# AuCson/DSP-Speech-Recognition

Hardware: NVIDIA B200
Metric: audio-sec/sec of MFCC+delta+pitch+endpoint (full front-end), ragged 0.5-5 s utterances, per-GPU LPT shards (higher is better)
Workload: dtype f32

## Files before the change

### dsp-speech-recognition_b200/csrc/fft_regs.h

```cpp
#pragma once
#include "simt.h"

namespace dspfe {

struct cpx2 { float2 re, im; };

DEVFN cpx2 cadd(cpx2 a, cpx2 b) { cpx2 r; r.re = f2add(a.re, b.re); r.im = f2add(a.im, b.im); return r; }
DEVFN cpx2 csub(cpx2 a, cpx2 b) { cpx2 r; r.re = f2sub(a.re, b.re); r.im = f2sub(a.im, b.im); return r; }
DEVFN cpx2 cmuls(cpx2 a, float wr, float wi) {
    cpx2 r;
    r.re = f2fmas(a.re, wr, f2muls(a.im, -wi));
    r.im = f2fmas(a.re, wi, f2muls(a.im, wr));
    return r;
}
DEVFN cpx2 cmul_negi(cpx2 a) { cpx2 r; r.re = a.im; r.im = f2neg(a.re); return r; }

DEVFN void dft4(cpx2& a, cpx2& b, cpx2& c, cpx2& d) {
    cpx2 t0 = cadd(a, c), t1 = csub(a, c), t2 = cadd(b, d), t3 = cmul_negi(csub(b, d));
    a = cadd(t0, t2); c = csub(t0, t2); b = cadd(t1, t3); d = csub(t1, t3);
}

DEVFN void dft16(cpx2 (&x)[16]) {
    const float c1 = 0.92387953251128674f, s1 = 0.38268343236508977f, r2 = 0.70710678118654752f;
#pragma unroll
    for (int nb = 0; nb < 4; ++nb) dft4(x[nb], x[4 + nb], x[8 + nb], x[12 + nb]);
    x[5] = cmuls(x[5], c1, -s1);
    { cpx2 t = x[6]; x[6].re = f2muls(f2add(t.re, t.im), r2); x[6].im = f2muls(f2sub(t.im, t.re), r2); }
    x[7] = cmuls(x[7], s1, -c1);
    { cpx2 t = x[9]; x[9].re = f2muls(f2add(t.re, t.im), r2); x[9].im = f2muls(f2sub(t.im, t.re), r2); }
    x[10] = cmul_negi(x[10]);
    { cpx2 t = x[11]; x[11].re = f2muls(f2sub(t.im, t.re), r2); x[11].im = f2muls(f2add(t.re, t.im), -r2); }
    x[13] = cmuls(x[13], s1, -c1);
    { cpx2 t = x[14]; x[14].re = f2muls(f2sub(t.im, t.re), r2); x[14].im = f2muls(f2add(t.re, t.im), -r2); }
    x[15] = cmuls(x[15], -c1, s1);
#pragma unroll
    for (int ka = 0; ka < 4; ++ka) dft4(x[4 * ka], x[4 * ka + 1], x[4 * ka + 2], x[4 * ka + 3]);
#pragma unroll
    for (int a = 0; a < 4; ++a)
#pragma unroll
        for (int b = a + 1; b < 4; ++b) { cpx2 t = x[4 * a + b]; x[4 * a + b] = x[4 * b + a]; x[4 * b + a] = t; }
}

DEVFN cpx2 shfl_xor_c(cpx2 a, int m) {
    cpx2 r;
    r.re.x = simt::shfl32_xor(a.re.x, m); r.re.y = simt::shfl32_xor(a.re.y, m);
    r.im.x = simt::shfl32_xor(a.im.x, m); r.im.y = simt::shfl32_xor(a.im.y, m);
    return r;
}

template <bool W32IMM = false>
DEVFN void fft512(cpx2 (&x)[16], float2* scr, const float2* tws, const float2* w32s, int lane) {
    dft16(x);
    const int q = lane >> 4, ll = lane & 15;
    const float sg = q ? -1.f : 1.f;
#pragma unroll
    for (int k1 = 0; k1 < 16; ++k1) {
        const float kC[16] = {1.0f, 0.98078528f, 0.923879533f, 0.831469612f, 0.707106781f, 0.555570233f, 0.382683432f, 0.195090322f, 6.123234e-17f, -0.195090322f, -0.382683432f, -0.555570233f, -0.707106781f, -0.831469612f, -0.923879533f, -0.98078528f};
        const float kS[16] = {-0.0f, -0.195090322f, -0.382683432f, -0.555570233f, -0.707106781f, -0.831469612f, -0.923879533f, -0.98078528f, -1.0f, -0.98078528f, -0.923879533f, -0.831469612f, -0.707106781f, -0.555570233f, -0.382683432f, -0.195090322f};
        const float2 w = W32IMM ? make_float2(q ? kC[k1] : 1.f, q ? kS[k1] : 0.f) : w32s[2 * k1 + q];
        const cpx2 u = cmuls(x[k1], w.x, w.y);
        const cpx2 v = shfl_xor_c(u, 16);
        cpx2 d; d.re = f2fmas(u.re, sg, v.re); d.im = f2fmas(u.im, sg, v.im);
        const float2 t = tws[k1 * 32 + lane];
        x[k1] = cmuls(d, t.x, t.y);
    }
    float2* tile = scr + q * (16 * 17);
#pragma unroll
    for (int k1 = 0; k1 < 16; ++k1) tile[k1 * 17 + ll] = x[k1].re;
    simt::warp_sync();
#pragma unroll
    for (int n2 = 0; n2 < 16; ++n2) x[n2].re = tile[ll * 17 + n2];
    simt::warp_sync();
#pragma unroll
    for (int k1 = 0; k1 < 16; ++k1) tile[k1 * 17 + ll] = x[k1].im;
    simt::warp_sync();
#pragma unroll
    for (int n2 = 0; n2 < 16; ++n2) x[n2].im = tile[ll * 17 + n2];
    simt::warp_sync();
    dft16(x);
}

}
```

### dsp-speech-recognition_b200/csrc/pitch_kernel.cuh

```cuda
#pragma once
#include <math.h>
#include <stdint.h>

#include "simt.h"
#include "fft_regs.h"
#ifndef DSPFE_EMU
#include <cuda_fp16.h>
#endif

#ifndef DSP_HD
#ifdef __CUDACC__
#define DSP_HD __host__ __device__ inline
#else
#define DSP_HD inline
#endif
#endif

namespace dspfe {

constexpr int kPitchFft = 1024;
constexpr int kCepLen = 512;
constexpr int kCepCols = 200;
constexpr int kAcrLags = 180;
constexpr int kMinLag = 20;
// ... 398 lines not shown
    int u, nf; int64_t g0;
    slot_unit(p, h0, kClipRun, lane, u, g0, nf);
    if (lane == 0) p.run_desc[h0 / kClipRun] = make_int4((int)(g0 & 0xffffffffll), (int)(g0 >> 32), nf, u);
    if (nf == 0) return;
    const int Ld = p.ds_len[u];
    const int kf0 = (int)(g0 - p.frame_off[u]) * step;
    const int fit = ((kClipDecCap - L) / step + 1) & ~1;
#pragma unroll 1
    for (int j0 = 0; j0 < nf; j0 += fit) {
        const int nj = nf - j0 < fit ? nf - j0 : fit;
        const int span = (nj - 1) * step + L;
        simt::warp_sync();
        FrameCursor c = frame_cursor(p, g0 + j0, u, lane, true, stage, span, kClipStageBytes);
        const int rows = (((span + 31) >> 5) + 3) & ~3;
        const bool pre = p.pre_hi != 0.f || p.pre_lo != 0.f;
        if (p.in_f32) { if (pre) decimate_span<true, true>(p, c, ds_idx, dec, lane, rows); else decimate_span<true, false>(p, c, ds_idx, dec, lane, rows); }
        else { if (pre) decimate_span<false, true>(p, c, ds_idx, dec, lane, rows); else decimate_span<false, false>(p, c, ds_idx, dec, lane, rows); }
        simt::warp_sync();
#pragma unroll 1
        for (int j = j0; j < j0 + nj; j += 2) {
            const bool hasB = j + 1 < nf && j + 1 < j0 + nj;
            float xa[NT], xb[NT], fa = 0.f, fb = 0.f;
            const int base = (j - j0) * step;
            const int cnta = L < Ld - (kf0 + j * step) ? L : Ld - (kf0 + j * step);
            const int cntb = hasB ? (L < Ld - (kf0 + (j + 1) * step) ? L : Ld - (kf0 + (j + 1) * step)) : 0;
#pragma unroll
            for (int t = 0; t < NT; ++t) {
                const int n = 32 * t + lane;
                const float va = n < cnta ? dec[base + n] : 0.f, vb = n < cntb ? dec[base + step + n] : 0.f;
                xa[t] = va; xb[t] = vb; fa += fabsf(va); fb += fabsf(vb);
            }
            if (p.frame_amp) {
                double sa = (double)fa, sb = (double)fb;
#pragma unroll
                for (int m = 16; m >= 1; m >>= 1) { sa += shfl32_xor_f64(sa, m); sb += shfl32_xor_f64(sb, m); }
                if (lane == 0) { p.frame_amp[g0 + j] = sa; if (hasB) p.frame_amp[g0 + j + 1] = sb; }
            }
            float2 med = make_float2(0.f, 0.f);
            if (p.do_clip) med = I16 ? warp_median_nonneg2_i16<NT>(xa, xb, L, lane) : warp_median_nonneg2<NT>(xa, xb, L, lane);
            float2* dst = p.clip + ((h0 + j) >> 1) * 512;
#pragma unroll
            for (int t = 0; t < 16; ++t) {
                float2 o = make_float2(0.f, 0.f);
                if (t < NT && lane + 32 * t < L) {
                    o.x = p.do_clip ? clip_value(xa[t < NT ? t : 0], med.x) : xa[t < NT ? t : 0];
                    o.y = p.do_clip ? clip_value(xb[t < NT ? t : 0], med.y) : xb[t < NT ? t : 0];
                }
                dst[32 * t + lane] = o;
            }
        }
    }
}

template <int MODE>
DEVFN void pitch_fft_pair(const PitchParams& p, int64_t h0, int64_t g0, bool hasB, unsigned char* wsm, const float2* tws, const float2* w32s) {
    const int lane = simt::tid() & 31;
    float2* scr = reinterpret_cast<float2*>(wsm);
    float4* park = reinterpret_cast<float4*>(scr + kWarpScr);
    float2* xs = p.clip + (h0 >> 1) * 512;
    const float2* modA = p.tab + kTabMod;
    const float2* HeB = p.tab + kTabHe;
    const float2* HoB = p.tab + kTabHo;
    const int L = p.frame_len;
    cpx2 x[16];
    const float2 zero2 = make_float2(0.f, 0.f);
    const float inv1024 = 1.0f / 1024.0f;
    constexpr int kStages = MODE == 0 ? 5 : 8;
#pragma unroll 1
    for (int st = 0; st < kStages; ++st) {
        const bool inv = MODE == 0 ? (st == 2 || st == 4) : (st & 1);
        const bool load = MODE == 0 ? st <= 1 : !(st & 1);
        const bool loadmod = MODE == 0 ? st == 1 : (st == 2 || st == 6);
        if (load) {
#pragma unroll
            for (int t = 0; t < 16; ++t) {
                const float2 xv = xs[32 * t + lane];
                float2 m = make_float2(1.f, 0.f);
                if (loadmod) m = ldg(modA + 32 * t + lane);
                x[t].re = f2muls(xv, m.x); x[t].im = f2muls(xv, m.y);
            }
        }
        if (inv) {
#pragma unroll
            for (int t = 0; t < 16; ++t) x[t].im = f2neg(x[t].im);
        }
        fft512<true>(x, scr, tws, w32s, lane);
        if (inv) {
#pragma unroll
            for (int t = 0; t < 16; ++t) x[t].im = f2neg(x[t].im);
        }
        const bool mulH = MODE == 0 ? st <= 1 : (st == 0 || st == 2);
        const bool mulM = MODE == 0 ? st == 2 : st == 3;
        if (mulH || mulM) {
            const float2* T = mulM ? modA : ((MODE == 0 ? st == 0 : st == 0) ? HeB : HoB);
            const float sr = mulM ? (MODE == 0 ? inv1024 : 1.f) : ((MODE == 0 && st == 0) ? 0.5f : 1.f);
            const float si = mulM ? -sr : sr;
#pragma unroll
            for (int t = 0; t < 16; ++t) { const float2 h = ldg(T + 32 * t + lane); x[t] = cmuls(x[t], h.x * sr, h.y * si); }
        }
        if (MODE == 0) {
            if (st == 0) {
#pragma unroll
                for (int t = 0; t < 16; ++t) park[32 * t + lane] = make_float4(x[t].re.x, x[t].re.y, x[t].im.x, x[t].im.y);
            } else if (st == 3) {
#pragma unroll
                for (int t = 0; t < 16; ++t) {
                    const float4 pk = park[32 * t + lane];
                    const float2 yr = f2add(x[t].re, make_float2(pk.x, pk.y)), yi = f2add(x[t].im, make_float2(pk.z, pk.w));
                    const float2 s2 = f2fma(yi, yi, f2mul(yr, yr));
                    x[t].re = make_float2(0.5f * dsp_fast_logf(s2.x), 0.5f * dsp_fast_logf(s2.y));
                    x[t].im = zero2;
                }
            } else if (st == 4) {
                const float inv512 = 1.0f / 512.0f;
                float* rowa = p.rows + g0 * p.row_len;
                float* rowb = rowa + p.row_len;
#pragma unroll
                for (int t = 0; t < 16; ++t) {
                    const int n = 32 * t + lane;
                    if (n < p.row_len) {
                        const float2 s2 = f2fma(x[t].im, x[t].im, f2mul(x[t].re, x[t].re));
                        rowa[n] = dsp_fast_sqrtf(s2.x) * inv512;
                        if (hasB) rowb[n] = dsp_fast_sqrtf(s2.y) * inv512;
                    }
                }
            }
        } else {
            if (st == 1) {
#pragma unroll
                for (int t = 0; t < 16; ++t) park[32 * t + lane] = make_float4(x[t].re.x, x[t].re.y, x[t].im.x, x[t].im.y);
            } else if (st == 3) {
#pragma unroll
                for (int t = 0; t < 16; ++t) {
                    const float4 pk = park[32 * t + lane];
                    const float2 yr = f2add(x[t].re, make_float2(pk.x, pk.y)), yi = f2add(x[t].im, make_float2(pk.z, pk.w));
                    const float2 s2 = f2fma(yi, yi, f2mul(yr, yr));
                    const bool in = 32 * t + lane < L;
                    xs[32 * t + lane] = make_float2(in ? dsp_fast_sqrtf(s2.x) * inv1024 : 0.f, in ? dsp_fast_sqrtf(s2.y) * inv1024 : 0.f);
                }
            } else if (st == 4 || st == 6) {
#pragma unroll
                for (int t = 0; t < 16; ++t) { x[t].re = f2fma(x[t].im, x[t].im, f2mul(x[t].re, x[t].re)); x[t].im = zero2; }
// ... 95 lines not shown
            for (int t = 0; t < kQuadT; ++t) {
                const float2 s2 = f2fma(x[t].im, x[t].im, f2mul(x[t].re, x[t].re));
                const bool in = 32 * t + lane < L;
                v[t] = make_float2(in ? dsp_fast_sqrtf(s2.x) : 0.f, in ? dsp_fast_sqrtf(s2.y) : 0.f);
            }
            if (st == 1) {
#pragma unroll
                for (int t = 0; t < kQuadT; ++t) vpark[32 * t + lane] = v[t];
            } else {
                float2 e1 = zero2, e2 = zero2;
#pragma unroll
                for (int t = 0; t < kQuadT; ++t) { const float2 a = vpark[32 * t + lane]; x[t].re = a; e1 = f2fma(a, a, e1); e2 = f2fma(v[t], v[t], e2); }
#pragma unroll
                for (int m = 16; m >= 1; m >>= 1) {
                    e1.x += simt::shfl32_xor(e1.x, m); e1.y += simt::shfl32_xor(e1.y, m);
                    e2.x += simt::shfl32_xor(e2.x, m); e2.y += simt::shfl32_xor(e2.y, m);
                }
                int kx = ((__float_as_int_compat(e1.x) >> 23) - (__float_as_int_compat(e2.x) >> 23)) / 2;
                int ky = ((__float_as_int_compat(e1.y) >> 23) - (__float_as_int_compat(e2.y) >> 23)) / 2;
                if (!(e1.x > 0.f && e2.x > 0.f && e1.x < 3e38f && e2.x < 3e38f)) kx = 0;
                if (!(e1.y > 0.f && e2.y > 0.f && e1.y < 3e38f && e2.y < 3e38f)) ky = 0;
                kx = kx < -40 ? -40 : (kx > 40 ? 40 : kx); ky = ky < -40 ? -40 : (ky > 40 ? 40 : ky);
                const float2 sc2 = make_float2(__int_as_float_compat((127 + kx) << 23), __int_as_float_compat((127 + ky) << 23));
                unscale = make_float2(__int_as_float_compat((127 - 2 * kx) << 23), __int_as_float_compat((127 - 2 * ky) << 23));
#pragma unroll
                for (int t = 0; t < 16; ++t) {
                    if (t >= kQuadT) x[t].re = zero2;
                    x[t].im = t < kQuadT ? f2mul(v[t < kQuadT ? t : 0], sc2) : zero2;
                }
            }
        } else if (st == 4) {
            split_pairs<1>(x, tabA, tabB, lane);
        } else {
            const float inv512 = 1.0f / 512.0f;
            float* row = p.rows + g0 * p.row_len;
            const int RL = p.row_len;
            const bool f1 = nvalid > 1, f2 = nvalid > 2, f3 = nvalid > 3;
#pragma unroll
            for (int t = 0; t < 7; ++t) {
                const int n = 32 * t + lane, j = n - kMinLag;
                if (j >= 0 && j < RL) {
                    const float sc = (n < L) ? inv512 / (float)(L - n) : NAN;
                    row[j] = x[t].re.x * sc;
                    if (f1) row[RL + j] = x[t].re.y * sc;
                    if (f2) row[2 * RL + j] = -x[t].im.x * unscale.x * sc;
                    if (f3) row[3 * RL + j] = -x[t].im.y * unscale.y * sc;
                }
            }
        }
    }
}

constexpr int kTrackListPerWarp = kTrackChunk * kPeakLags / (kTrackThreads / 32);
DEVFN bool stops(float x, float v) { return !(x <= v); }

DEVFN void pitch_track_cta(const PitchParams& p, float* buf, int* sc, double* spitch) {
    const int u = p.order ? p.order[simt::bid()] : simt::bid();
    const int tid = simt::tid();
    const int lane = tid & 31, warp = tid >> 5;
    const int64_t f0 = p.frame_off[u];
    const int F = (int)(p.frame_off[u + 1] - f0);
    const int RL = p.row_len;
    const int CH = track_chunk(RL);
    const float* rows = p.rows + f0 * RL;
    spitch = reinterpret_cast<double*>((reinterpret_cast<uintptr_t>(spitch) + 7) & ~(uintptr_t)7);
    int32_t* slag = reinterpret_cast<int32_t*>(spitch + kTrackMaxFrames);
    unsigned short* olist = reinterpret_cast<unsigned short*>(slag + kTrackMaxFrames);
    const bool staged = F <= kTrackMaxFrames;
    int32_t* lagv = staged ? slag : p.lag + f0;
    float s1[2] = {0.f, 0.f}, s2[2] = {0.f, 0.f};
    for (int c0 = 0; c0 < F; c0 += CH) {
        const int nrows = F - c0 < CH ? F - c0 : CH;
        const int nload = (c0 + nrows < F ? nrows + 1 : nrows) * RL;
        const float* src = rows + (int64_t)c0 * RL;
        if ((RL & 3) == 0 && ((reinterpret_cast<uintptr_t>(src) & 15) == 0)) {
            const int n4 = nload >> 2;
            for (int i0 = tid; i0 < n4; i0 += 8 * kTrackThreads) {
                float4 v[8];
#pragma unroll
                for (int k = 0; k < 8; ++k) { const int i = i0 + k * kTrackThreads; if (i < n4) v[k] = ldg(reinterpret_cast<const float4*>(src) + i); }
#pragma unroll
                for (int k = 0; k < 8; ++k) { const int i = i0 + k * kTrackThreads; if (i < n4) reinterpret_cast<float4*>(buf)[i] = v[k]; }
            }
        } else {
            for (int i = tid; i < nload; i += kTrackThreads) buf[i] = src[i];
        }
        simt::cta_sync();
        if (!p.no_smooth) {
#pragma unroll
            for (int cc = 0; cc < 2; ++cc) {
                const int col = tid + cc * kTrackThreads;
                if (col < RL) {
                    float a2 = s2[cc], a1 = s1[cc];
                    float r0 = buf[col];
                    for (int k = 0; k < nrows; ++k) {
                        const int i = c0 + k;
                        float gsm, r1 = 0.f;
                        if (i >= 2 && i + 2 < F) {
                            r1 = buf[(k + 1) * RL + col];
                            gsm = (((a2 + a1) + r0) + r1) * 0.25f;
                        } else {
                            const int right = (i + 2 < F) ? i + 2 : F - 1;
                            const int left = i - 2 > 0 ? i - 2 : 0;
                            float acc = 0.f; bool any = false;
                            if (i - 2 >= 0 && i - 2 < right) { acc = a2; any = true; }
                            if (i - 1 >= 0 && i - 1 < right) { acc = any ? acc + a1 : a1; any = true; }
                            if (i < right) { acc = any ? acc + r0 : r0; any = true; }
                            if (i + 1 < F) r1 = buf[(k + 1) * RL + col];
                            if (i + 1 < right) { acc = any ? acc + r1 : r1; any = true; }
                            gsm = any ? acc / (float)(right - left) : NAN;
                        }
                        buf[k * RL + col] = gsm;
                        if (p.rows_out) p.rows_out[(f0 + i) * RL + col] = gsm;
                        a2 = a1; a1 = gsm; r0 = r1;
                    }
                    s2[cc] = a2; s1[cc] = a1;
                }
            }
        } else if (p.rows_out) {
            for (int i = tid; i < nrows * RL; i += kTrackThreads) p.rows_out[(f0 + c0) * RL + i] = buf[i];
        }
        simt::cta_sync();
        if (p.mode == 0) {
            const int ntask = nrows * kPeakLags;
            unsigned short* wlist = olist + warp * kTrackListPerWarp;
            int n_open = 0;
            const bool wide = RL >= kMinLag + kPeakLags + 4;
            for (int t0 = warp * 32; t0 < ntask; t0 += kTrackThreads) {
                const int t = t0 + lane;
                const bool live = t < ntask;
                const int k = live ? t / kPeakLags : 0, c = kMinLag + (live ? t % kPeakLags : 0);
                const float* row = buf + k * RL;
                const float v = row[c];
                const int rmax = c < RL - c ? c : RL - c;
                int sv;
                if (wide) {
                    const bool s1 = stops(row[c - 1], v) || stops(row[c + 1], v), s2 = stops(row[c - 2], v) || stops(row[c + 2], v);
                    const bool s3 = stops(row[c - 3], v) || stops(row[c + 3], v), s4 = stops(row[c - 4], v) || stops(row[c + 4], v);
                    sv = s1 ? 1 : (s2 ? 2 : (s3 ? 3 : (s4 ? 4 : 5)));
                    sv = sv < rmax ? sv : rmax;
                } else {
                    int r = 1;
                    while (r < rmax && r <= 4 && !stops(row[c - r], v) && !stops(row[c + r], v)) ++r;
                    sv = r;
                }
                if (!(v == v)) sv = 0;
                const bool is_open = live && sv > 4 && sv < rmax;
                if (live) sc[t] = sv;
                const unsigned m = simt::ballot32(is_open);
                if (is_open) wlist[n_open + dsp_popc(m & ((1u << lane) - 1u))] = (unsigned short)t;
                n_open += dsp_popc(m);
            }
            simt::warp_sync();
            for (int i0 = 0; i0 < n_open; i0 += 32) {
                const bool has = i0 + lane < n_open;
                const int t = has ? wlist[i0 + lane] : 0;
                const int k = t / kPeakLags, c = kMinLag + t % kPeakLags;
                const float* row = buf + k * RL;
                const float v = row[c];
                const int rmax = c < RL - c ? c : RL - c;
                int found = -1, r = 5;
                bool pending = has;
#pragma unroll 1
                for (int round = 0; round < 4 && simt::ballot32(pending) != 0; ++round, r += 8) {
                    int first = 8;
#pragma unroll
                    for (int d = 7; d >= 0; --d) {
                        const int rr = r + d < rmax ? r + d : rmax - 1;
                        const bool st = r + d < rmax && (stops(row[c - rr], v) || stops(row[c + rr], v));
                        first = st ? d : first;
                    }
                    if (pending) {
                        if (first < 8) { found = r + first; pending = false; }
                        else if (r + 8 >= rmax) { found = rmax; pending = false; }
                    }
                }
                unsigned todo = simt::ballot32(pending);
                while (todo) {
                    const int src = __builtin_ffs((int)todo) - 1;
                    todo &= todo - 1;
                    const int ck = simt::shfl32_i(k, src), cc = simt::shfl32_i(c, src), cm = simt::shfl32_i(rmax, src);
                    const float cv = __int_as_float_compat(simt::shfl32_i(__float_as_int_compat(v), src));
                    const float* crow = buf + ck * RL;
                    int f = cm;
                    for (int r0 = 37; r0 < cm; r0 += 32) {
                        const int rr = r0 + lane;
                        const bool st = rr < cm && (stops(crow[cc - rr], cv) || stops(crow[cc + rr], cv));
                        const unsigned hit = simt::ballot32(st);
                        if (hit) { f = r0 + __builtin_ffs((int)hit) - 1; break; }
                    }
                    if (lane == src) found = f;
                }
                if (has) sc[t] = found;
            }
            simt::cta_sync();
            for (int k = warp; k < nrows; k += kTrackThreads / 32) {
                const int* srow = sc + k * kPeakLags;
                if (p.score) for (int t = lane; t < kPeakLags; t += 32) p.score[(f0 + c0 + k) * kPeakLags + t] = srow[t];
                unsigned key = 0;
                for (int t = lane; t < kPeakLags; t += 32) { const unsigned q = ((unsigned)srow[t] << 7) | (unsigned)(127 - t); key = q > key ? q : key; }
                key = warp_redux_max(key);
                if (lane == 0) lagv[c0 + k] = kMinLag + 127 - (int)(key & 127u);
            }
        } else {
            for (int k = warp; k < nrows; k += kTrackThreads / 32) {
                const float* row = buf + k * RL;
                unsigned best = 0;
                for (int j = lane; j < RL; j += 32) {
                    const float v = row[j];
                    const unsigned b = (unsigned)__float_as_int_compat(v);
                    const unsigned q = v != v ? 0xffffffffu : (b ^ ((b >> 31) ? 0xffffffffu : 0x80000000u));
                    best = q > best ? q : best;
                }
                const unsigned top = warp_redux_max(best);
                unsigned idx = 0xffffffffu;
                for (int j = lane; j < RL; j += 32) {
                    const float v = row[j];
                    const unsigned b = (unsigned)__float_as_int_compat(v);
                    const unsigned q = v != v ? 0xffffffffu : (b ^ ((b >> 31) ? 0xffffffffu : 0x80000000u));
                    if (q == top && (unsigned)j < idx) idx = (unsigned)j;
                }
                idx = warp_redux_min(idx);
                if (lane == 0) lagv[c0 + k] = kMinLag + (int)idx;
            }
        }
        simt::cta_sync();
    }
    if (!staged) {
        if (tid == 0 && F > 0 && p.pitch) robust_pitch(p.lag + f0, F, p.pitch + f0);
        return;
    }
    for (int i = tid; i < F; i += kTrackThreads) spitch[i] = 1.0 / (0.0001 * (double)slag[i]);
    simt::cta_sync();
    if (tid == 0 && p.pitch) {
        for (int i = 1; i < F; ++i)
            if (fabs(2 * spitch[i] - spitch[i - 1]) < 50 && spitch[i] < 170) spitch[i] = 2 * spitch[i];
        for (int i = F - 2; i > 0; --i)
            if (fabs(2 * spitch[i] - spitch[i + 1]) < 50 && spitch[i] < 170) spitch[i] = 2 * spitch[i];
    }
    simt::cta_sync();
    for (int i = tid; i < F; i += kTrackThreads) {
        p.lag[f0 + i] = slag[i];
        if (p.pitch) p.pitch[f0 + i] = spitch[i];
    }
}

constexpr int kFeatMaxFrames = 640;
DEVFN double warp_kth(const double* v, int n, int k, int lane) {
    double out = 0.0; int found = 0;
    for (int e = lane; e < n; e += 32) {
        const double x = v[e];
        int rank = 0;
        for (int j = 0; j < n; ++j) rank += (v[j] < x || (v[j] == x && j < e)) ? 1 : 0;
        if (rank == k) { out = x; found = 1; }
    }
    const int src = __builtin_ffs((int)simt::ballot32(found != 0)) - 1;
    return shfl32_f64(out, src);
}
DEVFN void pitch_feature_warp(const PitchParams& p, int u, double* sm) {
    const int lane = simt::tid() & 31;
    const int64_t f0 = p.frame_off[u];
    const int F = (int)(p.frame_off[u + 1] - f0);
    double* out5 = p.feat + 5 * (int64_t)u;
    if (F > kFeatMaxFrames) {
        if (lane == 0) pitch_feature_tail(p.pitch + f0, p.frame_amp + f0, F, p.scratch + 3 * f0, out5);
        return;
    }
    double* pitch = sm; double* amp = sm + kFeatMaxFrames; double* s1 = amp + kFeatMaxFrames; double* s2 = s1 + kFeatMaxFrames;
    double* tmp = s2 + kFeatMaxFrames;
    for (int i = lane; i < F; i += 32) { pitch[i] = p.pitch[f0 + i]; amp[i] = p.frame_amp[f0 + i]; }
    simt::warp_sync();
    double bs = -1000.0; int bi = 0;
    for (int i = 10 + lane; i < F - 10; i += 32) {
        bool lower = false;
        for (int j = i - 2; j <= i + 2; ++j) lower = lower || (amp[j] < amp[i]);
        if (lower) continue;
        double sc = 0;
        for (int j = i - 10; j <= i + 10; ++j) sc += amp[j] - amp[i];
        if (sc > bs) { bs = sc; bi = i; }
    }
// ... 30 lines not shown
```

### dsp-speech-recognition_b200/csrc/simt.h

```cpp
#pragma once
#include <stdint.h>

#ifdef DSPFE_EMU
#include <cmath>
#include <cstring>
struct float2 { float x, y; };
struct float4 { float x, y, z, w; };
static inline float2 make_float2(float x, float y) { float2 r; r.x = x; r.y = y; return r; }
static inline float4 make_float4(float x, float y, float z, float w) { float4 r; r.x = x; r.y = y; r.z = z; r.w = w; return r; }
#define DEVFN static inline
#define DSPFE_RESTRICT
namespace simt {
int tid();
int bid();
int nthreads();
void cta_sync();
void group_sync();
float shfl16(float v, int src);
float shfl32_xor(float v, int m);
int shfl32_i(int v, int src);
unsigned ballot32(bool pred);
void warp_sync();
struct mbar_t { uint64_t v; };
static inline void mbar_init(mbar_t*, int) {}
static inline void fence_mbar_init() {}
static inline void fence_proxy_async() {}
static inline void mbar_expect_tx(mbar_t*, uint32_t) {}
static inline void bulk_g2s(void* dst, const void* src, uint32_t bytes, mbar_t*) { std::memcpy(dst, src, bytes); }
static inline void mbar_wait(mbar_t*, uint32_t) {}
}
DEVFN float2 f2add(float2 a, float2 b) { return make_float2(a.x + b.x, a.y + b.y); }
DEVFN float2 f2sub(float2 a, float2 b) { return make_float2(a.x - b.x, a.y - b.y); }
DEVFN float2 f2mul(float2 a, float2 b) { return make_float2(a.x * b.x, a.y * b.y); }
DEVFN float2 f2fma(float2 a, float2 b, float2 c) { return make_float2(std::fmaf(a.x, b.x, c.x), std::fmaf(a.y, b.y, c.y)); }
DEVFN float dsp_logf(float x) { return std::log(x); }
static inline float sqrtf_(float x) { return std::sqrt(x); }
DEVFN float dsp_fmaf(float a, float b, float c) { return std::fmaf(a, b, c); }
DEVFN float dsp_fast_logf(float x) { return std::log(x); }
DEVFN float dsp_fast_sqrtf(float x) { return std::sqrt(x); }
DEVFN float cvt_i16(int v) { return (float)v; }
template <class T> DEVFN T ldg(const T* p) { return *p; }
DEVFN float cvt_lo16(uint32_t w) { return (float)(int16_t)(w & 0xffffu); }
DEVFN float cvt_hi16(uint32_t w) { return (float)(int16_t)(w >> 16); }
struct uint4 { uint32_t x, y, z, w; };
struct int4 { int x, y, z, w; };
static inline uint4 make_uint4(uint32_t x, uint32_t y, uint32_t z, uint32_t w) { uint4 r; r.x = x; r.y = y; r.z = z; r.w = w; return r; }
static inline int4 make_int4(int x, int y, int z, int w) { int4 r; r.x = x; r.y = y; r.z = z; r.w = w; return r; }
#else
#include <cuda_runtime.h>
#define DEVFN __device__ __forceinline__
#define DSPFE_RESTRICT __restrict__
namespace simt {
DEVFN int tid() { return threadIdx.x; }
DEVFN int bid() { return blockIdx.x; }
DEVFN int nthreads() { return blockDim.x; }
DEVFN void cta_sync() { __syncthreads(); }
DEVFN void group_sync() { __syncwarp(); }
DEVFN float shfl16(float v, int src) { return __shfl_sync(0xffffffffu, v, src, 16); }
DEVFN float shfl32_xor(float v, int m) { return __shfl_xor_sync(0xffffffffu, v, m); }
DEVFN int shfl32_i(int v, int src) { return __shfl_sync(0xffffffffu, v, src); }
DEVFN unsigned ballot32(bool pred) { return __ballot_sync(0xffffffffu, pred); }
DEVFN void warp_sync() { __syncwarp(); }

struct mbar_t { uint64_t v; };
DEVFN uint32_t smem_u32(const void* p) { return (uint32_t)__cvta_generic_to_shared(p); }
DEVFN void mbar_init(mbar_t* b, int count) {
    asm volatile("mbarrier.init.shared::cta.b64 [%0], %1;" ::"r"(smem_u32(b)), "r"(count));
}
DEVFN void fence_mbar_init() { asm volatile("fence.mbarrier_init.release.cluster;" ::: "memory"); }
DEVFN void fence_proxy_async() { asm volatile("fence.proxy.async.shared::cta;" ::: "memory"); }
DEVFN void mbar_expect_tx(mbar_t* b, uint32_t bytes) {
    asm volatile("mbarrier.arrive.expect_tx.shared::cta.b64 _, [%0], %1;" ::"r"(smem_u32(b)), "r"(bytes) : "memory");
}
DEVFN void bulk_g2s(void* dst, const void* src, uint32_t bytes, mbar_t* b) {
    asm volatile("cp.async.bulk.shared::cluster.global.mbarrier::complete_tx::bytes [%0], [%1], %2, [%3];"
                 ::"r"(smem_u32(dst)), "l"(src), "r"(bytes), "r"(smem_u32(b)) : "memory");
}
DEVFN void mbar_wait(mbar_t* b, uint32_t parity) {
    asm volatile(
        "{\n\t.reg .pred p;\n\t"
        "WAIT_%=:\n\t"
        "mbarrier.try_wait.parity.shared::cta.b64 p, [%0], %1;\n\t"
        "@p bra DONE_%=;\n\t"
        "bra WAIT_%=;\n\t"
        "DONE_%=:\n\t}" ::"r"(smem_u32(b)), "r"(parity) : "memory");
}
}
DEVFN float2 f2add(float2 a, float2 b) { return __fadd2_rn(a, b); }
DEVFN float2 f2sub(float2 a, float2 b) { return __fadd2_rn(a, make_float2(-b.x, -b.y)); }
DEVFN float2 f2mul(float2 a, float2 b) { return __fmul2_rn(a, b); }
DEVFN float2 f2fma(float2 a, float2 b, float2 c) { return __ffma2_rn(a, b, c); }
DEVFN float dsp_logf(float x) { return logf(x); }
DEVFN float dsp_fmaf(float a, float b, float c) { return fmaf(a, b, c); }
DEVFN float dsp_fast_logf(float x) { return __logf(x); }
DEVFN float dsp_fast_sqrtf(float x) { float r; asm("sqrt.approx.f32 %0, %1;" : "=f"(r) : "f"(x)); return r; }
DEVFN float cvt_i16(int v) { return __uint_as_float(0x4B000000u | (((unsigned)v & 0xffffu) ^ 0x8000u)) - 8421376.0f; }
template <class T> DEVFN T ldg(const T* p) { return __ldg(p); }
DEVFN float cvt_lo16(uint32_t w) { return __uint_as_float(__byte_perm(w ^ 0x80008000u, 0x4B000000u, 0x7610)) - 8421376.0f; }
DEVFN float cvt_hi16(uint32_t w) { return __uint_as_float(__byte_perm(w ^ 0x80008000u, 0x4B000000u, 0x7632)) - 8421376.0f; }
#endif

#ifdef DSPFE_EMU
DEVFN int __float_as_int_compat(float f) { int i; std::memcpy(&i, &f, 4); return i; }
DEVFN float __int_as_float_compat(int i) { float f; std::memcpy(&f, &i, 4); return f; }
#else
DEVFN int __float_as_int_compat(float f) { return __float_as_int(f); }
DEVFN float __int_as_float_compat(int i) { return __int_as_float(i); }
#endif

DEVFN int dsp_popc(unsigned v) {
#ifdef DSPFE_EMU
    return __builtin_popcount(v);
#else
    return __popc(v);
#endif
}

DEVFN int warp_redux_add(int v) {
#ifdef DSPFE_EMU
    for (int m = 16; m >= 1; m >>= 1) v += simt::shfl32_i(v, (simt::tid() & 31) ^ m);
    return v;
#else
    return __reduce_add_sync(0xffffffffu, v);
#endif
}
DEVFN unsigned warp_redux_min(unsigned v) {
#ifdef DSPFE_EMU
    for (int m = 16; m >= 1; m >>= 1) { const unsigned o = (unsigned)simt::shfl32_i((int)v, (simt::tid() & 31) ^ m); v = o < v ? o : v; }
    return v;
// ... 49 lines not shown
```

Measured before the change: 1.665 million.

## Use packed-real FFT trick for final pitch stage with dynamic range scaling

For the last pitch FFT stage (MODE 0, stage 4), the two frames' real-valued data are packed as one complex signal and run through a single 512-point FFT. The spectra are then separated with a conjugate-symmetric split via lane shuffles, which roughly halves the FFT arithmetic and shuffle work for that stage. To keep f32 accuracy, each half is scaled by a power of two to equalise exponents, with a fallback to the old path when magnitudes are too large. The FFT helpers are templated on a new single-complex type so both paths share code. The cost is a warp-wide max reduction, a branch and extra register pressure.

After: 1.687 million, median of 6. +1.3%, better.

```diff
diff --git a/dsp-speech-recognition_b200/csrc/fft_regs.h b/dsp-speech-recognition_b200/csrc/fft_regs.h
--- a/dsp-speech-recognition_b200/csrc/fft_regs.h
+++ b/dsp-speech-recognition_b200/csrc/fft_regs.h
@@ -4,6 +4,7 @@
 namespace dspfe {
 
 struct cpx2 { float2 re, im; };
+struct cpx1 { float2 z; };
 
 DEVFN cpx2 cadd(cpx2 a, cpx2 b) { cpx2 r; r.re = f2add(a.re, b.re); r.im = f2add(a.im, b.im); return r; }
 DEVFN cpx2 csub(cpx2 a, cpx2 b) { cpx2 r; r.re = f2sub(a.re, b.re); r.im = f2sub(a.im, b.im); return r; }
@@ -14,31 +15,49 @@
     return r;
 }
 DEVFN cpx2 cmul_negi(cpx2 a) { cpx2 r; r.re = a.im; r.im = f2neg(a.re); return r; }
+DEVFN cpx2 cmul_w2(cpx2 t, float r2) { cpx2 r; r.re = f2muls(f2add(t.re, t.im), r2); r.im = f2muls(f2sub(t.im, t.re), r2); return r; }
+DEVFN cpx2 cmul_w6(cpx2 t, float r2) { cpx2 r; r.re = f2muls(f2sub(t.im, t.re), r2); r.im = f2muls(f2add(t.re, t.im), -r2); return r; }
+DEVFN cpx2 cfmas(cpx2 a, float s, cpx2 b) { cpx2 r; r.re = f2fmas(a.re, s, b.re); r.im = f2fmas(a.im, s, b.im); return r; }
 
-DEVFN void dft4(cpx2& a, cpx2& b, cpx2& c, cpx2& d) {
-    cpx2 t0 = cadd(a, c), t1 = csub(a, c), t2 = cadd(b, d), t3 = cmul_negi(csub(b, d));
+DEVFN cpx1 cadd(cpx1 a, cpx1 b) { cpx1 r; r.z = f2add(a.z, b.z); return r; }
+DEVFN cpx1 csub(cpx1 a, cpx1 b) { cpx1 r; r.z = f2sub(a.z, b.z); return r; }
+DEVFN cpx1 cmuls(cpx1 a, float wr, float wi) {
+    cpx1 r;
+    r.z.x = dsp_fmaf(a.z.x, wr, -a.z.y * wi);
+    r.z.y = dsp_fmaf(a.z.x, wi, a.z.y * wr);
+    return r;
+}
+DEVFN cpx1 cmul_negi(cpx1 a) { cpx1 r; r.z = make_float2(a.z.y, -a.z.x); return r; }
+DEVFN cpx1 cmul_w2(cpx1 t, float r2) { cpx1 r; r.z = make_float2((t.z.x + t.z.y) * r2, (t.z.y - t.z.x) * r2); return r; }
+DEVFN cpx1 cmul_w6(cpx1 t, float r2) { cpx1 r; r.z = make_float2((t.z.y - t.z.x) * r2, (t.z.x + t.z.y) * -r2); return r; }
+DEVFN cpx1 cfmas(cpx1 a, float s, cpx1 b) { cpx1 r; r.z = f2fmas(a.z, s, b.z); return r; }
+
+template <class T>
+DEVFN void dft4(T& a, T& b, T& c, T& d) {
+    T t0 = cadd(a, c), t1 = csub(a, c), t2 = cadd(b, d), t3 = cmul_negi(csub(b, d));
     a = cadd(t0, t2); c = csub(t0, t2); b = cadd(t1, t3); d = csub(t1, t3);
 }
 
-DEVFN void dft16(cpx2 (&x)[16]) {
+template <class T>
+DEVFN void dft16(T (&x)[16]) {
     const float c1 = 0.92387953251128674f, s1 = 0.38268343236508977f, r2 = 0.70710678118654752f;
 #pragma unroll
     for (int nb = 0; nb < 4; ++nb) dft4(x[nb], x[4 + nb], x[8 + nb], x[12 + nb]);
     x[5] = cmuls(x[5], c1, -s1);
-    { cpx2 t = x[6]; x[6].re = f2muls(f2add(t.re, t.im), r2); x[6].im = f2muls(f2sub(t.im, t.re), r2); }
+    x[6] = cmul_w2(x[6], r2);
     x[7] = cmuls(x[7], s1, -c1);
-    { cpx2 t = x[9]; x[9].re = f2muls(f2add(t.re, t.im), r2); x[9].im = f2muls(f2sub(t.im, t.re), r2); }
+    x[9] = cmul_w2(x[9], r2);
     x[10] = cmul_negi(x[10]);
-    { cpx2 t = x[11]; x[11].re = f2muls(f2sub(t.im, t.re), r2); x[11].im = f2muls(f2add(t.re, t.im), -r2); }
+    x[11] = cmul_w6(x[11], r2);
     x[13] = cmuls(x[13], s1, -c1);
-    { cpx2 t = x[14]; x[14].re = f2muls(f2sub(t.im, t.re), r2); x[14].im = f2muls(f2add(t.re, t.im), -r2); }
+    x[14] = cmul_w6(x[14], r2);
     x[15] = cmuls(x[15], -c1, s1);
 #pragma unroll
     for (int ka = 0; ka < 4; ++ka) dft4(x[4 * ka], x[4 * ka + 1], x[4 * ka + 2], x[4 * ka + 3]);
 #pragma unroll
     for (int a = 0; a < 4; ++a)
 #pragma unroll
-        for (int b = a + 1; b < 4; ++b) { cpx2 t = x[4 * a + b]; x[4 * a + b] = x[4 * b + a]; x[4 * b + a] = t; }
+        for (int b = a + 1; b < 4; ++b) { T t = x[4 * a + b]; x[4 * a + b] = x[4 * b + a]; x[4 * b + a] = t; }
 }
 
 DEVFN cpx2 shfl_xor_c(cpx2 a, int m) {
@@ -47,23 +66,9 @@
     r.im.x = simt::shfl32_xor(a.im.x, m); r.im.y = simt::shfl32_xor(a.im.y, m);
     return r;
 }
+DEVFN cpx1 shfl_xor_c(cpx1 a, int m) { cpx1 r; r.z.x = simt::shfl32_xor(a.z.x, m); r.z.y = simt::shfl32_xor(a.z.y, m); return r; }
 
-template <bool W32IMM = false>
-DEVFN void fft512(cpx2 (&x)[16], float2* scr, const float2* tws, const float2* w32s, int lane) {
-    dft16(x);
-    const int q = lane >> 4, ll = lane & 15;
-    const float sg = q ? -1.f : 1.f;
-#pragma unroll
-    for (int k1 = 0; k1 < 16; ++k1) {
-        const float kC[16] = {1.0f, 0.98078528f, 0.923879533f, 0.831469612f, 0.707106781f, 0.555570233f, 0.382683432f, 0.195090322f, 6.123234e-17f, -0.195090322f, -0.382683432f, -0.555570233f, -0.707106781f, -0.831469612f, -0.923879533f, -0.98078528f};
-        const float kS[16] = {-0.0f, -0.195090322f, -0.382683432f, -0.555570233f, -0.707106781f, -0.831469612f, -0.923879533f, -0.98078528f, -1.0f, -0.98078528f, -0.923879533f, -0.831469612f, -0.707106781f, -0.555570233f, -0.382683432f, -0.195090322f};
-        const float2 w = W32IMM ? make_float2(q ? kC[k1] : 1.f, q ? kS[k1] : 0.f) : w32s[2 * k1 + q];
-        const cpx2 u = cmuls(x[k1], w.x, w.y);
-        const cpx2 v = shfl_xor_c(u, 16);
-        cpx2 d; d.re = f2fmas(u.re, sg, v.re); d.im = f2fmas(u.im, sg, v.im);
-        const float2 t = tws[k1 * 32 + lane];
-        x[k1] = cmuls(d, t.x, t.y);
-    }
+DEVFN void tile_transpose(cpx2 (&x)[16], float2* scr, int q, int ll) {
     float2* tile = scr + q * (16 * 17);
 #pragma unroll
     for (int k1 = 0; k1 < 16; ++k1) tile[k1 * 17 + ll] = x[k1].re;
@@ -77,6 +82,34 @@
 #pragma unroll
     for (int n2 = 0; n2 < 16; ++n2) x[n2].im = tile[ll * 17 + n2];
     simt::warp_sync();
+}
+DEVFN void tile_transpose(cpx1 (&x)[16], float2* scr, int q, int ll) {
+    float2* tile = scr + q * (16 * 17);
+#pragma unroll
+    for (int k1 = 0; k1 < 16; ++k1) tile[k1 * 17 + ll] = x[k1].z;
+    simt::warp_sync();
+#pragma unroll
+    for (int n2 = 0; n2 < 16; ++n2) x[n2].z = tile[ll * 17 + n2];
+    simt::warp_sync();
+}
+
+template <bool W32IMM = false, class T>
+DEVFN void fft512(T (&x)[16], float2* scr, const float2* tws, const float2* w32s, int lane) {
+    dft16(x);
+    const int q = lane >> 4, ll = lane & 15;
+    const float sg = q ? -1.f : 1.f;
+#pragma unroll
+    for (int k1 = 0; k1 < 16; ++k1) {
+        const float kC[16] = {1.0f, 0.98078528f, 0.923879533f, 0.831469612f, 0.707106781f, 0.555570233f, 0.382683432f, 0.195090322f, 6.123234e-17f, -0.195090322f, -0.382683432f, -0.555570233f, -0.707106781f, -0.831469612f, -0.923879533f, -0.98078528f};
+        const float kS[16] = {-0.0f, -0.195090322f, -0.382683432f, -0.555570233f, -0.707106781f, -0.831469612f, -0.923879533f, -0.98078528f, -1.0f, -0.98078528f, -0.923879533f, -0.831469612f, -0.707106781f, -0.555570233f, -0.382683432f, -0.195090322f};
+        const float2 w = W32IMM ? make_float2(q ? kC[k1] : 1.f, q ? kS[k1] : 0.f) : w32s[2 * k1 + q];
+        const T u = cmuls(x[k1], w.x, w.y);
+        const T v = shfl_xor_c(u, 16);
+        const T d = cfmas(u, sg, v);
+        const float2 t = tws[k1 * 32 + lane];
+        x[k1] = cmuls(d, t.x, t.y);
+    }
+    tile_transpose(x, scr, q, ll);
     dft16(x);
 }
 
diff --git a/dsp-speech-recognition_b200/csrc/pitch_kernel.cuh b/dsp-speech-recognition_b200/csrc/pitch_kernel.cuh
--- a/dsp-speech-recognition_b200/csrc/pitch_kernel.cuh
+++ b/dsp-speech-recognition_b200/csrc/pitch_kernel.cuh
@@ -474,6 +474,55 @@
     }
 }
 
+DEVFN bool real_pair_scale(cpx1 (&z)[16], float2& us) {
+    unsigned ma = 0, mb = 0;
+#pragma unroll
+    for (int t = 0; t < 16; ++t) {
+        const unsigned a = (unsigned)__float_as_int_compat(z[t].z.x) & 0x7fffffffu, b = (unsigned)__float_as_int_compat(z[t].z.y) & 0x7fffffffu;
+        ma = a > ma ? a : ma; mb = b > mb ? b : mb;
+    }
+    ma = warp_redux_max(ma); mb = warp_redux_max(mb);
+    const unsigned kBig = 0x71800000u;
+    if (ma >= kBig || mb >= kBig) return false;
+    int k = (ma != 0 && mb != 0) ? (int)(ma >> 23) - (int)(mb >> 23) : 0;
+    k = k < -120 ? -120 : (k > 120 ? 120 : k);
+    const float up = __int_as_float_compat((127 + (k < 0 ? -k : k)) << 23), down = __int_as_float_compat((127 - (k < 0 ? -k : k)) << 23);
+    const float2 sc = k < 0 ? make_float2(up, 1.f) : make_float2(1.f, up);
+    us = k < 0 ? make_float2(down, 1.f) : make_float2(1.f, down);
+#pragma unroll
+    for (int t = 0; t < 16; ++t) z[t].z = f2mul(z[t].z, sc);
+    return true;
+}
+DEVFN cpx1 shfl_c(cpx1 a, int src) {
+    cpx1 r;
+    r.z.x = __int_as_float_compat(simt::shfl32_i(__float_as_int_compat(a.z.x), src));
+    r.z.y = __int_as_float_compat(simt::shfl32_i(__float_as_int_compat(a.z.y), src));
+    return r;
+}
+DEVFN cpx2 split_real_one(cpx1 z, cpx1 r, float2 s) {
+    cpx2 o;
+    o.re = f2mul(f2add(z.z, r.z), s);
+    o.im = f2mul(make_float2(z.z.y - r.z.y, r.z.x - z.z.x), s);
+    return o;
+}
+template <int NP, bool BOTH>
+DEVFN void split_real_pair(const cpx1 (&z)[16], cpx2 (&x)[16], float2 s, int lane) {
+    const int src = (32 - lane) & 31;
+    const bool l0 = lane == 0;
+#pragma unroll
+    for (int t = 0; t < NP; ++t) {
+        const int a = t, b = 15 - t;
+        cpx1 ra = shfl_c(z[b], src);
+        if (l0) ra = z[(16 - a) & 15];
+        x[a] = split_real_one(z[a], ra, s);
+        if (BOTH) {
+            cpx1 rb = shfl_c(z[a], src);
+            if (l0) rb = z[a + 1];
+            x[b] = split_real_one(z[b], rb, s);
+        }
+    }
+}
+
 template <int MODE>
 DEVFN void pitch_fft_pair(const PitchParams& p, int64_t h0, int64_t g0, bool hasB, unsigned char* wsm, const float2* tws, const float2* w32s) {
     const int lane = simt::tid() & 31;
@@ -493,23 +542,39 @@
         const bool inv = MODE == 0 ? (st == 2 || st == 4) : (st & 1);
         const bool load = MODE == 0 ? st <= 1 : !(st & 1);
         const bool loadmod = MODE == 0 ? st == 1 : (st == 2 || st == 6);
-        if (load) {
-#pragma unroll
-            for (int t = 0; t < 16; ++t) {
-                const float2 xv = xs[32 * t + lane];
-                float2 m = make_float2(1.f, 0.f);
-                if (loadmod) m = ldg(modA + 32 * t + lane);
-                x[t].re = f2muls(xv, m.x); x[t].im = f2muls(xv, m.y);
-            }
-        }
-        if (inv) {
-#pragma unroll
-            for (int t = 0; t < 16; ++t) x[t].im = f2neg(x[t].im);
-        }
-        fft512<true>(x, scr, tws, w32s, lane);
-        if (inv) {
-#pragma unroll
-            for (int t = 0; t < 16; ++t) x[t].im = f2neg(x[t].im);
+        bool split = false;
+        if (MODE == 0 && st == 4) {
+            cpx1 z[16];
+#pragma unroll
+            for (int t = 0; t < 16; ++t) z[t].z = x[t].re;
+            float2 us;
+            split = real_pair_scale(z, us);
+            if (split) {
+                fft512<true>(z, scr, tws, w32s, lane);
+                us = f2muls(us, 0.5f);
+                if (p.row_len > 7 * 32) split_real_pair<8, true>(z, x, us, lane);
+                else split_real_pair<7, false>(z, x, us, lane);
+            }
+        }
+        if (!split) {
+            if (load) {
+#pragma unroll
+                for (int t = 0; t < 16; ++t) {
+                    const float2 xv = xs[32 * t + lane];
+                    float2 m = make_float2(1.f, 0.f);
+                    if (loadmod) m = ldg(modA + 32 * t + lane);
+                    x[t].re = f2muls(xv, m.x); x[t].im = f2muls(xv, m.y);
+                }
+            }
+            if (inv) {
+#pragma unroll
+                for (int t = 0; t < 16; ++t) x[t].im = f2neg(x[t].im);
+            }
+            fft512<true>(x, scr, tws, w32s, lane);
+            if (inv) {
+#pragma unroll
+                for (int t = 0; t < 16; ++t) x[t].im = f2neg(x[t].im);
+            }
         }
         const bool mulH = MODE == 0 ? st <= 1 : (st == 0 || st == 2);
         const bool mulM = MODE == 0 ? st == 2 : st == 3;
```

## Overlap pitch-track score argmax with next chunk load and prefetch chunks to L2

Applied to the files above, without the earlier changes.

In the pitch tracking kernel, the per-row score argmax for a chunk is deferred so it runs while the next chunk is being staged into shared memory. This drops one CTA barrier per chunk, and the last chunk is handled after the loop. Thread 0 issues a bulk L2 prefetch of the next chunk's rows. The autocorrelation argmax becomes a single pass that tracks the first index of the maximum. Compile-time phase gates and a phase-profiling script are added; the default of 6 keeps the full behaviour. Deferring the argmax relies on the score buffer not being overwritten before it is read, which adds a correctness risk.

Measured after the change: 1.660 million before, 1.684 million after, median of 6. 1.01x the previous value.

```diff
diff --git a/dsp-speech-recognition_b200/csrc/pitch_kernel.cuh b/dsp-speech-recognition_b200/csrc/pitch_kernel.cuh
--- a/dsp-speech-recognition_b200/csrc/pitch_kernel.cuh
+++ b/dsp-speech-recognition_b200/csrc/pitch_kernel.cuh
@@ -711,6 +711,10 @@
 }
 
 constexpr int kTrackListPerWarp = kTrackChunk * kPeakLags / (kTrackThreads / 32);
+#ifndef DSPFE_TRACK_PHASES
+#define DSPFE_TRACK_PHASES 6
+#endif
+constexpr int kTrackPhases = DSPFE_TRACK_PHASES;
 DEVFN bool stops(float x, float v) { return !(x <= v); }
 
 DEVFN void pitch_track_cta(const PitchParams& p, float* buf, int* sc, double* spitch) {
@@ -728,10 +732,26 @@
     const bool staged = F <= kTrackMaxFrames;
     int32_t* lagv = staged ? slag : p.lag + f0;
     float s1[2] = {0.f, 0.f}, s2[2] = {0.f, 0.f};
+    auto chunk_floats = [&](int c) { const int n = F - c < CH ? F - c : CH; return (c + n < F ? n + 1 : n) * RL; };
+    auto score_argmax = [&](int c, int nrows) {
+        for (int k = warp; k < nrows && kTrackPhases >= 5; k += kTrackThreads / 32) {
+            const int* srow = sc + k * kPeakLags;
+            if (p.score) for (int t = lane; t < kPeakLags; t += 32) p.score[(f0 + c + k) * kPeakLags + t] = srow[t];
+            unsigned key = 0;
+            for (int t = lane; t < kPeakLags; t += 32) { const unsigned q = ((unsigned)srow[t] << 7) | (unsigned)(127 - t); key = q > key ? q : key; }
+            key = warp_redux_max(key);
+            if (lane == 0) lagv[c + k] = kMinLag + 127 - (int)(key & 127u);
+        }
+    };
     for (int c0 = 0; c0 < F; c0 += CH) {
         const int nrows = F - c0 < CH ? F - c0 : CH;
-        const int nload = (c0 + nrows < F ? nrows + 1 : nrows) * RL;
+        const int nload = chunk_floats(c0);
         const float* src = rows + (int64_t)c0 * RL;
+        if (tid == 0 && c0 + CH < F) {
+            const uintptr_t a = reinterpret_cast<uintptr_t>(src + (int64_t)CH * RL) & ~(uintptr_t)15;
+            const uintptr_t e = reinterpret_cast<uintptr_t>(src + (int64_t)CH * RL + chunk_floats(c0 + CH)) & ~(uintptr_t)15;
+            if (e > a) simt::prefetch_l2(reinterpret_cast<const void*>(a), (uint32_t)(e - a));
+        }
         if ((RL & 3) == 0 && ((reinterpret_cast<uintptr_t>(src) & 15) == 0)) {
             const int n4 = nload >> 2;
             for (int i0 = tid; i0 < n4; i0 += 8 * kTrackThreads) {
@@ -744,8 +764,9 @@
         } else {
             for (int i = tid; i < nload; i += kTrackThreads) buf[i] = src[i];
         }
+        if (p.mode == 0 && c0 > 0) score_argmax(c0 - CH, CH);
         simt::cta_sync();
-        if (!p.no_smooth) {
+        if (!p.no_smooth && kTrackPhases >= 1) {
 #pragma unroll
             for (int cc = 0; cc < 2; ++cc) {
                 const int col = tid + cc * kTrackThreads;
@@ -780,7 +801,7 @@
             for (int i = tid; i < nrows * RL; i += kTrackThreads) p.rows_out[(f0 + c0) * RL + i] = buf[i];
         }
         simt::cta_sync();
-        if (p.mode == 0) {
+        if (p.mode == 0 && kTrackPhases >= 2) {
             const int ntask = nrows * kPeakLags;
             unsigned short* wlist = olist + warp * kTrackListPerWarp;
             int n_open = 0;
@@ -811,7 +832,7 @@
                 n_open += dsp_popc(m);
             }
             simt::warp_sync();
-            for (int i0 = 0; i0 < n_open; i0 += 32) {
+            for (int i0 = 0; i0 < n_open && kTrackPhases >= 3; i0 += 32) {
                 const bool has = i0 + lane < n_open;
                 const int t = has ? wlist[i0 + lane] : 0;
                 const int k = t / kPeakLags, c = kMinLag + t % kPeakLags;
@@ -834,7 +855,7 @@
                         else if (r + 8 >= rmax) { found = rmax; pending = false; }
                     }
                 }
-                unsigned todo = simt::ballot32(pending);
+                unsigned todo = kTrackPhases >= 4 ? simt::ballot32(pending) : 0u;
                 while (todo) {
                     const int src = __builtin_ffs((int)todo) - 1;
                     todo &= todo - 1;
@@ -852,39 +873,29 @@
                 }
                 if (has) sc[t] = found;
             }
-            simt::cta_sync();
-            for (int k = warp; k < nrows; k += kTrackThreads / 32) {
-                const int* srow = sc + k * kPeakLags;
-                if (p.score) for (int t = lane; t < kPeakLags; t += 32) p.score[(f0 + c0 + k) * kPeakLags + t] = srow[t];
-                unsigned key = 0;
-                for (int t = lane; t < kPeakLags; t += 32) { const unsigned q = ((unsigned)srow[t] << 7) | (unsigned)(127 - t); key = q > key ? q : key; }
-                key = warp_redux_max(key);
-                if (lane == 0) lagv[c0 + k] = kMinLag + 127 - (int)(key & 127u);
-            }
-        } else {
+        } else if (p.mode != 0 && kTrackPhases >= 5) {
             for (int k = warp; k < nrows; k += kTrackThreads / 32) {
                 const float* row = buf + k * RL;
-                unsigned best = 0;
+                unsigned best = 0, first = 0xffffffffu;
                 for (int j = lane; j < RL; j += 32) {
                     const float v = row[j];
                     const unsigned b = (unsigned)__float_as_int_compat(v);
                     const unsigned q = v != v ? 0xffffffffu : (b ^ ((b >> 31) ? 0xffffffffu : 0x80000000u));
-                    best = q > best ? q : best;
+                    if (q > best) { best = q; first = (unsigned)j; }
                 }
                 const unsigned top = warp_redux_max(best);
-                unsigned idx = 0xffffffffu;
-                for (int j = lane; j < RL; j += 32) {
-                    const float v = row[j];
-                    const unsigned b = (unsigned)__float_as_int_compat(v);
-                    const unsigned q = v != v ? 0xffffffffu : (b ^ ((b >> 31) ? 0xffffffffu : 0x80000000u));
-                    if (q == top && (unsigned)j < idx) idx = (unsigned)j;
-                }
-                idx = warp_redux_min(idx);
+                const unsigned idx = warp_redux_min(best == top ? first : 0xffffffffu);
                 if (lane == 0) lagv[c0 + k] = kMinLag + (int)idx;
             }
         }
         simt::cta_sync();
     }
+    if (p.mode == 0 && F > 0) {
+        const int last = (F - 1) / CH * CH;
+        score_argmax(last, F - last);
+        simt::cta_sync();
+    }
+    if (kTrackPhases < 6) return;
     if (!staged) {
         if (tid == 0 && F > 0 && p.pitch) robust_pitch(p.lag + f0, F, p.pitch + f0);
         return;
diff --git a/dsp-speech-recognition_b200/csrc/simt.h b/dsp-speech-recognition_b200/csrc/simt.h
--- a/dsp-speech-recognition_b200/csrc/simt.h
+++ b/dsp-speech-recognition_b200/csrc/simt.h
@@ -28,6 +28,7 @@
 static inline void mbar_expect_tx(mbar_t*, uint32_t) {}
 static inline void bulk_g2s(void* dst, const void* src, uint32_t bytes, mbar_t*) { std::memcpy(dst, src, bytes); }
 static inline void mbar_wait(mbar_t*, uint32_t) {}
+static inline void prefetch_l2(const void*, uint32_t) {}
 }
 DEVFN float2 f2add(float2 a, float2 b) { return make_float2(a.x + b.x, a.y + b.y); }
 DEVFN float2 f2sub(float2 a, float2 b) { return make_float2(a.x - b.x, a.y - b.y); }
@@ -75,6 +76,9 @@
 DEVFN void bulk_g2s(void* dst, const void* src, uint32_t bytes, mbar_t* b) {
     asm volatile("cp.async.bulk.shared::cluster.global.mbarrier::complete_tx::bytes [%0], [%1], %2, [%3];"
                  ::"r"(smem_u32(dst)), "l"(src), "r"(bytes), "r"(smem_u32(b)) : "memory");
+}
+DEVFN void prefetch_l2(const void* src, uint32_t bytes) {
+    asm volatile("cp.async.bulk.prefetch.L2.global [%0], %1;" ::"l"(src), "r"(bytes) : "memory");
 }
 DEVFN void mbar_wait(mbar_t* b, uint32_t parity) {
     asm volatile(
diff --git a/profiles/run_track_phases.py b/profiles/run_track_phases.py
--- /dev/null
+++ b/profiles/run_track_phases.py
@@ -0,0 +1,122 @@
+import argparse
+import concurrent.futures as cf
+import ctypes
+import importlib.util
+import json
+import os
+import subprocess
+import sys
+import tempfile
+
+import numpy as np
+
+HERE = os.path.dirname(os.path.abspath(__file__))
+ROOT = os.path.dirname(HERE)
+
+
+def build_variants(root, phases, tmp):
+    pkg = os.path.join(root, "dsp-speech-recognition_b200")
+    spec = importlib.util.spec_from_file_location("dspfe_build_variants", os.path.join(pkg, "build.py"))
+    b = importlib.util.module_from_spec(spec)
+    spec.loader.exec_module(b)
+    flags = [f for f in b.FLAGS if f not in ("-shared", "-Xptxas", "-v")]
+    srcs = b.sources()
+
+    def compile_one(src, obj, extra):
+        r = subprocess.run([b.NVCC] + flags + extra + ["-c", src, "-o", obj], capture_output=True, text=True)
+        if r.returncode:
+            raise RuntimeError(r.stdout + r.stderr)
+        return obj
+
+    jobs = {}
+    with cf.ThreadPoolExecutor(max_workers=max(2, os.cpu_count() or 2)) as ex:
+        for s in srcs:
+            name = os.path.splitext(os.path.basename(s))[0]
+            if name == "pitch":
+                for n in phases:
+                    jobs[("pitch", n)] = ex.submit(compile_one, s, os.path.join(tmp, f"pitch_p{n}.o"), [f"-DDSPFE_TRACK_PHASES={n}"])
+            else:
+                jobs[(name, None)] = ex.submit(compile_one, s, os.path.join(tmp, f"{name}.o"), [])
+        objs = {k: f.result() for k, f in jobs.items()}
+    common = [o for (name, n), o in objs.items() if name != "pitch"]
+    libs = {}
+    for n in phases:
+        lib = os.path.join(tmp, f"libdspfe_p{n}.so")
+        r = subprocess.run([b.NVCC, "-gencode", "arch=compute_100a,code=sm_100a", "-shared", "-o", lib, objs[("pitch", n)]] + common,
+                           capture_output=True, text=True)
+        if r.returncode:
+            raise RuntimeError(r.stdout + r.stderr)
+        libs[n] = lib
+    return libs
+
+
+def main(root, phases, rounds, out):
+    sys.path.insert(0, os.path.join(root, "dsp-speech-recognition_b200"))
+    import torch
+    import dspfe
+    from dspfe import binding, synth
+    spec = importlib.util.spec_from_file_location("bench_split", os.path.join(ROOT, "bench.py"))
+    bench = importlib.util.module_from_spec(spec)
+    spec.loader.exec_module(bench)
+
+    assert torch.cuda.is_available(), "run_track_phases.py needs a CUDA device"
+    dev = torch.device("cuda:0")
+    lengths = synth.ragged_lengths(4096, seed=2024)
+    pcm, off = synth.synth_batch_torch(lengths, seed0=555, device=dev)
+    off_np, off_d = off.numpy(), off.to(dev)
+    with tempfile.TemporaryDirectory() as tmp:
+        libs = build_variants(root, phases, tmp)
+        arms = {}
+        for n, path in libs.items():
+            binding._lib, binding._LIB_PATH = None, path
+            L = binding.lib()
+            fe = dspfe.FrontendPlan(delta_n=2)
+            arms[n] = (L, fe, fe.alloc(int(pcm.numel()), len(lengths), device=dev))
+
+        def step(n):
+            L, fe, o = arms[n]
+            binding._lib = L
+            fe.run(pcm, off_d, off_np, o)
+            return L
+
+        for n in phases:
+            for _ in range(3):
+                step(n)
+        torch.cuda.synchronize()
+        ms = {n: {"pitch_cep": [], "pitch_acr": []} for n in phases}
+        for _ in range(rounds):
+            for n in phases:
+                step(n)
+                dspfe.timing_begin()
+                step(n)
+                paths = bench.split_paths(dspfe.timing_end())
+                for path in ("pitch_cep", "pitch_acr"):
+                    ms[n][path].append(paths[path].get("pitch_track_kernel", 0.0))
+        for n in phases:
+            arms[n][1].close()
+        binding._lib = None
+    gpu = subprocess.run(["nvidia-smi", "--query-gpu=name,power.limit,clocks.max.sm", "--format=csv,noheader"],
+                         capture_output=True, text=True).stdout.strip().splitlines()
+    names = {0: "staging", 1: "smoothing", 2: "peak A", 3: "peak B", 4: "peak C", 5: "arg-max", 6: "octave repair + stores"}
+    res = {"gpu": gpu[0] if gpu else "unknown", "root": os.path.basename(os.path.abspath(root)), "utterances": len(lengths),
+           "rounds": rounds, "note": "pitch_track_kernel ms per step with the kernel stopped after each phase (median of rounds)",
+           "phases": {}}
+    for n in phases:
+        res["phases"][f"{n} {names[n]}"] = {p: {"median": round(float(np.median(v)), 4), "min": round(min(v), 4), "max": round(max(v), 4)}
+                                            for p, v in ms[n].items()}
+    line = json.dumps(res)
+    print(line)
+    if out:
+        os.makedirs(os.path.dirname(os.path.abspath(out)), exist_ok=True)
+        with open(out, "w") as f:
+            f.write(line + "\n")
+
+
+if __name__ == "__main__":
+    ap = argparse.ArgumentParser(description=__doc__, formatter_class=argparse.RawDescriptionHelpFormatter)
+    ap.add_argument("--root", default=ROOT, help="checkout whose csrc/ is built (default: this one)")
+    ap.add_argument("--phases", default="0,1,2,3,4,5,6")
+    ap.add_argument("--rounds", type=int, default=5)
+    ap.add_argument("--out", default=None, help="also write the JSON line to this file")
+    a = ap.parse_args()
+    main(a.root, [int(x) for x in a.phases.split(",")], a.rounds, a.out)
```
